# WU-CVGL/CasualHDRSplat

Measured on AMD Instinct MI355X. Metric: train-step images/sec (fwd+bwd raster) @ 1M Gaussians 1080p, higher is better.
Workload: dtype f32; 1 GPU; c3: 1000000 Gaussians, 1920x1080, SH degree 3, HDR radiance + CRF tone-map, 1 pose(s)/view, 1 view(s)/step (one per GPU); num_rendered_R=6777809, R_prime=3025699, pixel_pair_evals_E=559372855, seed=0, binning=sync-free fixed capacity 1.25*R, launch=eager (one enqueue per kernel)

## Files before the change

### casualhdrsplat_amd/csrc/api.hip

```cpp
#include <stdarg.h>
#include <stdio.h>
#include <stdlib.h>
#include <string.h>
#include <time.h>
#include <unistd.h>
#include <atomic>

#include "hs_cloud.h"

namespace hs {

static thread_local char g_err[512] = "";

#ifdef HS_TESTING
int fault_injection() {
    static const int mode = [] {
        const char* e = getenv("HS_FAULT_INJECT");
        return (e && !strcmp(e, "sort_ticket")) ? 1 : (e && !strcmp(e, "stalled_chain")) ? 2 : (e && !strcmp(e, "late_block")) ? 3 : 0;
    }();
    return mode;
}
#endif

static std::atomic<int> g_sort_tickets{0};
// ... 51 lines not shown

void set_error(const char* fmt, ...) {
    va_list ap;
    va_start(ap, fmt);
    vsnprintf(g_err, sizeof g_err, fmt, ap);
    va_end(ap);
}

int64_t crf_partial_floats(int K, int64_t HW, int n_poses);
int64_t pose_partial_floats(int P, int N);

static int plan(const hs_dims& d, hs_sizes* sz, hs_layout* L) {
    if (d.P < 0 || d.W <= 0 || d.H <= 0 || d.n_poses < 1 || d.capacity < 0 || d.M < 0 || d.crf_K < 0 || d.crf_K > 4096 ||
        d.crf_K == 1 || d.n_poses > kMaxPoses) {
        set_error("hs_plan: bad dims P=%d W=%d H=%d N=%d capacity=%lld", d.P, d.W, d.H, d.n_poses, (long long)d.capacity);
        return HS_EINVAL;
    }
    if (d.n_frames < 0 || d.n_frames > d.n_poses || (d.n_frames > 1 && d.n_poses % d.n_frames != 0)) {
        set_error("hs_plan: n_frames=%d must lie in [0, n_poses=%d] and divide n_poses", d.n_frames, d.n_poses);
        return HS_EINVAL;
    }
    const int F = frames_of(d), npf = d.n_poses / F;
    const int64_t I = (int64_t)d.P * d.n_poses;
    const int64_t gx = (d.W + kTile - 1) / kTile, gy = (d.H + kTile - 1) / kTile;
    const int64_t vtiles = gx * gy * d.n_poses;
    if (I >= (1ll << 30) || vtiles >= (1ll << 31) || d.capacity >= (1ll << 30) || gx * gy >= (1ll << 22)) {
        set_error("hs_plan: problem too large (instances and binning capacity must stay below 2^30, tiles per pose below 2^22)");
        return HS_EINVAL;
    }
    const int64_t HW = (int64_t)d.W * d.H;
    hs_layout l;
    int64_t o = 0;
    auto carve = [&o](int64_t bytes) { int64_t at = o; o = align_up(o + bytes, 256); return at; };
    l.counters = carve(sizeof(hs_counters));
    l.rec = carve(I * kRecFloats * 4);
    l.depth = carve(I * 4);
    l.radii = carve(I * 4);
    l.tiles_touched = carve(I * 4);
    l.offsets = carve(I * 4);
    l.cov3D = carve((int64_t)d.P * 6 * 4);
    l.clamped = carve(I);
    l.scan_spine = carve(((I + 255) / 256 + 1) * 4);
    l.binfo = carve(I * 8);
    sz->geom_bytes = o;
    o = 0;
    l.keys_sorted = carve(2 * align_up(d.capacity * 4, 256));
    l.point_list = l.keys_sorted + align_up(d.capacity * 4, 256);
    l.pairs_tmp = carve(d.capacity * 8);
    l.ranges = carve(vtiles * 8);
    l.sort_tmp = carve(sort_tmp_bytes(I));
    l.depth_ws = carve(depth_ws_words(I) * 4);
    l.depth_pairs = carve(2 * I * 8);
    l.inst_sorted = carve(I * 4);
    l.offs_sorted = carve(I * 4);
    l.pair_sort_tmp = carve(emit_scan_words(I) * 4 + sort_tmp_bytes(d.capacity));
    l.pair_flags = carve(d.capacity);
    l.pair_act = carve(d.capacity);
    l.tile_matrix = carve(count_matrix_words(I, vtiles, d.capacity) * 4);
    l.hier_ws = carve(hier_ws_words(I, gx, gy, d.n_poses, d.capacity) * 4);
    sz->binning_bytes = o;
    o = 0;
    l.final_T = carve(HW * d.n_poses * 4);
    l.n_contrib = carve(HW * d.n_poses * 4);
    l.pose_hdr = carve(HW * 3 * 4 * (d.n_poses + (npf > 1 ? F : 0)));
    l.tile_work = carve(vtiles * 4);
    l.tile_order = carve(vtiles * 4);
    sz->image_bytes = o;
    o = 0;
    l.pair_grads = carve(d.capacity * kPairFloats * 4);
    l.crf_partials = carve(crf_partial_floats(d.crf_K, HW, d.n_poses) * 4);
    l.inst_grads = carve(I * kInstFloats * 4);
    l.pose_partials = carve(pose_partial_floats(d.P, d.n_poses) * 4);
    sz->bwd_bytes = o;
    if (L) *L = l;
    return HS_OK;
}

static int debug_sync(int flags, hipStream_t s, const char* stage) {
    if (!(flags & HS_FLAG_DEBUG)) return HS_OK;
    const hipError_t e = hipStreamSynchronize(s);
    if (e != hipSuccess) {
        set_error("debug: stage `%s` failed: %s", stage, hipGetErrorString(e));
        return HS_EHIP;
    }
    return HS_OK;
}

static int check_common(const hs_dims& d, const float* means3D, const float* shs, const float* colors,
                        const float* scales, const float* rots, const float* cov, const float* view,
                        const float* proj, const float* campos, const float* bg, const char* who) {
    if (!means3D || !view || !proj || !campos || !bg) { set_error("%s: null required pointer", who); return HS_EINVAL; }
    if ((shs == nullptr) == (colors == nullptr)) { set_error("%s: provide exactly one of shs / colors_precomp", who); return HS_EINVAL; }
    const bool sr = scales && rots;
    if (sr == (cov != nullptr) || ((scales == nullptr) != (rots == nullptr))) {
        set_error("%s: provide exactly one of (scales, rotations) / cov3D_precomp", who);
        return HS_EINVAL;
    }
    if (shs) {
        if (d.M > 32) {
            set_error("%s: M=%d SH coefficients per channel; at most 32 are supported", who, d.M);
            return HS_EINVAL;
        }
        if (d.sh_degree < 0 || d.sh_degree > 3 || (d.sh_degree + 1) * (d.sh_degree + 1) > d.M) {
            set_error("%s: sh_degree %d needs %d coefficients, M=%d", who, d.sh_degree, (d.sh_degree + 1) * (d.sh_degree + 1), d.M);
            return HS_EINVAL;
        }
    }
// ... 354 lines not shown
```

### casualhdrsplat_amd/csrc/binning.hip

```cpp
#include "hs_common.h"

#ifndef HS_EMIT_NT_MASK
#define HS_EMIT_NT_MASK 6
#endif

namespace hs {

namespace {

constexpr int kScanItems = 4;
constexpr int kScanTile = 256 * kScanItems;

__device__ __forceinline__ uint32_t wave_incl_scan(uint32_t v, int lane) {
#pragma unroll
    for (int d = 1; d < 64; d <<= 1) {
        uint32_t t = __shfl_up(v, d);
        if (lane >= d) v += t;
    }
    return v;
}

template <int NW = 4>
__device__ __forceinline__ uint32_t block_incl_scan(uint32_t v, uint32_t* s_wave , uint32_t* total) {
    const int lane = threadIdx.x & 63, wave = threadIdx.x >> 6;
// ... 1072 lines not shown
                        const int l = (int)__builtin_ctzll(missing);
                        missing &= missing - 1ull;
                        const int q = base - l;
                        uint32_t tot = 0;
                        for (int r = 0; r < 4; ++r) {
                            const int64_t ii = (int64_t)q * 256 + r * 64 + lane;
                            if (ii < I && counters->overflow < 2u) {
                                const uint2 rq = binfo[inst_sorted[ii]];
                                tot += (rq.y & 0xFFFFu) * (rq.y >> 16);
                            }
                        }
#pragma unroll
                        for (int d = 32; d >= 1; d >>= 1) tot += (uint32_t)__shfl_xor((int)tot, d);
                        if (lane == 0) {
                            atomicCAS(reinterpret_cast<unsigned long long*>(scan_status + q), 0ull, (unsigned long long)(kScAgg | (uint64_t)tot));
                            atomicAdd(&counters->reserved[4], 1u);
                        }
                    }
                }
                __builtin_amdgcn_s_sleep(1);
                if ((x & kScFlag) == 0ull) x = sc_read(scan_status + idx);
            }
            const uint64_t flag = x & kScFlag;
            poison = poison || __ballot(flag == 0ull || flag == kScPoison) != 0ull;
            const uint64_t incl_mask = __ballot(flag == kScIncl || flag == kScPoison || flag == 0ull);
            const int first = incl_mask ? (int)__builtin_ctzll(incl_mask) : 64;
            uint64_t v = lane <= first ? (x & ~kScFlag) : 0ull;
#pragma unroll
            for (int d = 32; d >= 1; d >>= 1) v += (uint64_t)__shfl_xor((long long)v, d);
            excl += v;
            if (incl_mask) break;
        }
        if (lane == 0) {
            if (blk != 0) sc_publish(scan_status + blk, (poison ? kScPoison : kScIncl) | ((excl + block_total) & ~kScFlag));
            s_excl = poison ? kScPoison : excl;
        }
    }
    __syncthreads();
    const bool poison = (s_excl & kScFlag) != 0ull;
    const uint64_t bexcl = s_excl & ~kScFlag;
    const uint64_t bend = bexcl + block_total;
    if (blk == (int)gridDim.x - 1 && threadIdx.x == 0) {
        const bool over = bend > capacity;
        counters->num_rendered = bend > 0xFFFFFFFFull ? 0xFFFFFFFFu : (uint32_t)bend;
        if (poison) counters->overflow = 2u;
        else if (over && counters->overflow < 2u) counters->overflow = 1u;
        counters->reserved[0] = (poison || over || counters->overflow != 0u) ? 0u : (uint32_t)bend;
        counters->reserved[5] = COUNT ? (uint32_t)kTileSortCount : (uint32_t)kTileSortRadix;
    }
    uint32_t beg = 0, end = 0;
    end = (uint32_t)bexcl + incl;
    beg = end - cnt;
    if (i < I) offs_sorted[i] = end;
    if (poison || bend > capacity) return;
    if (i < I && end > beg) {
        float* slot_start = &reinterpret_cast<float*>(rec + kRecF4 * (int64_t)inst + 2)[3];
        if constexpr (BIG && (HS_EMIT_NT_MASK & 2)) __builtin_nontemporal_store(__uint_as_float(beg), slot_start);
        else *slot_start = __uint_as_float(beg);
    }
    const uint32_t last_end = __shfl(end, 63 - __builtin_clzll(__ballot(i < I) | 1ull));
    if (i >= I) beg = end = last_end;
    {
        const uint32_t w = rc.y & 0xFFFFu;
        const uint32_t pose = I > (int64_t)P ? inst / (uint32_t)P : 0u;
        const uint32_t key0 = pose * (uint32_t)(gx * gy) + (rc.x >> 16) * (uint32_t)gx + (rc.x & 0xFFFFu);
        s_beg[wave][lane] = beg;
        s_own[wave][lane] = make_uint4(key0, w, __float_as_uint(1.0f / (float)w), inst);
    }
    int sh[4] = {0, 0, 0, 0}, wd[4] = {0, 0, 0, 0};
    {
        int shift = 0;
#pragma unroll
        for (int pass = 0; pass < 4; ++pass) {
            if (pass < passes) {
                const int w = (nbits - shift + (passes - pass) - 1) / (passes - pass);
                sh[pass] = shift; wd[pass] = w;
                shift += w;
            }
        }
    }
    const uint32_t first = __shfl(beg, 0);
    const uint32_t total = last_end - first;
    for (uint32_t p = lane; p < total; p += 64) {
        const uint32_t pos = first + p;
        uint32_t k = 0;
#pragma unroll
        for (uint32_t step = 32; step >= 1; step >>= 1)
            k |= (uint32_t)((int32_t)(s_beg[wave][k + step] - pos - 1u) >> 31) & step;
        const uint4 o = s_own[wave][k];
        const uint32_t t = pos - s_beg[wave][k];
        const uint32_t ty = (uint32_t)(((float)t + 0.5f) * __uint_as_float(o.z));
        const uint32_t tx = t - ty * o.y;
        const uint32_t key = o.x + ty * (uint32_t)gx + tx;
        if constexpr (BIG && (HS_EMIT_NT_MASK & 4)) { __builtin_nontemporal_store(key, &pairs[pos].x); __builtin_nontemporal_store(o.w, &pairs[pos].y); }
        else pairs[pos] = make_uint2(key, o.w);
        pair_flags[pos] = 0;
        if constexpr (COUNT) {
            atomicAdd(&s_hist[key], 1u << (8 * wave));
            continue;
        }
        const uint64_t act = __ballot(true);
#pragma unroll
        for (int pass = 0; pass < 4; ++pass) {
            if (pass < passes) {
                const uint32_t dgt = (key >> sh[pass]) & ((1u << wd[pass]) - 1u);
                const uint32_t d0 = __builtin_amdgcn_readfirstlane(dgt);
// ... 247 lines not shown
    for (int t = threadIdx.x; t < passes * 256; t += 256) s_dig[t] = 0;
    if (blockIdx.x == 0 && threadIdx.x < 2 * kDepthBitsCopies) depth_bits[threadIdx.x] = 0ull;
    const int wave = threadIdx.x >> 6, lane = threadIdx.x & 63;
    const int blk = blockIdx.x;
    const int64_t i = (int64_t)blk * 256 + threadIdx.x;
    uint32_t inst = 0;
    uint2 rc = make_uint2(0u, 0u);
    if (i < I && counters->overflow < 2u) { inst = inst_sorted[i]; rc = srect[i]; }
    const uint32_t cnt = (rc.y & 0xFFFFu) * (rc.y >> 16);
    uint32_t sx0, sy0, sw, sh;
    hier_coarse_rect(rc, sx0, sy0, sw, sh);
    const uint32_t ccnt = sw * sh;
    uint32_t block_total, block_ctotal;
    const uint32_t incl = block_incl_scan(cnt, s_wsum, &block_total);
    const uint32_t cincl = block_incl_scan(ccnt, s_wsum, &block_ctotal);
    if (excl_ready) {
        if (threadIdx.x == 0) { s_excl = block_excl[blk]; s_cexcl = block_cexcl[blk]; }
    } else {
        unsigned long long part = 0, cpart = 0;
        if (super_sums) {
            const int nsup = (HS_ABL & 8) ? 0 : blk / 4;
            for (int j = threadIdx.x; j < nsup; j += 256) { part += super_sums[j]; cpart += super_csums[j]; }
            if ((int)threadIdx.x < blk - 4 * (blk / 4)) { part += block_excl[4 * (blk / 4) + threadIdx.x]; cpart += block_cexcl[4 * (blk / 4) + threadIdx.x]; }
        } else {
            for (int j = threadIdx.x; j < ((HS_ABL & 8) ? 0 : blk); j += 256) { part += block_excl[j]; cpart += block_cexcl[j]; }
        }
#pragma unroll
        for (int d = 32; d >= 1; d >>= 1) {
            part += (unsigned long long)__shfl_xor((long long)part, d);
            cpart += (unsigned long long)__shfl_xor((long long)cpart, d);
        }
        if (lane == 0) { s_wsum64[wave] = part; s_beg[0][wave] = (uint32_t)cpart; }
        __syncthreads();
        if (threadIdx.x == 0) {
            s_excl = (s_wsum64[0] + s_wsum64[1]) + (s_wsum64[2] + s_wsum64[3]);
            s_cexcl = (s_beg[0][0] + s_beg[0][1]) + (s_beg[0][2] + s_beg[0][3]);
        }
    }
    __syncthreads();
    const uint64_t bexcl = s_excl;
    const uint64_t bend = bexcl + block_total;
    const uint32_t cbexcl = s_cexcl;
    if (blk == (int)gridDim.x - 1 && threadIdx.x == 0) {
        const bool over = bend > capacity;
        counters->num_rendered = bend > 0xFFFFFFFFull ? 0xFFFFFFFFu : (uint32_t)bend;
        if (over && counters->overflow < 2u) counters->overflow = 1u;
        const bool empty = over || counters->overflow != 0u;
        counters->reserved[0] = empty ? 0u : (uint32_t)bend;
        counters->reserved[5] = (uint32_t)kTileSortHier;
        hier[0] = empty ? 0u : cbexcl + block_ctotal;
    }
    const uint32_t end = (uint32_t)bexcl + incl, beg = end - cnt;
    if (i < I) offs_sorted[i] = end;
    if (bend > capacity) return;
    if (!(HS_ABL & 1) && i < I && end > beg) {
        float* slot_start = &reinterpret_cast<float*>(rec + kRecF4 * (int64_t)inst + 2)[3];
        if constexpr (BIG && (HS_HIER_NT_MASK & 2)) __builtin_nontemporal_store(__uint_as_float(beg), slot_start);
        else *slot_start = __uint_as_float(beg);
    }
    if (!(HS_ABL & 2)) {
        const uint64_t a0 = min(bend, (bexcl + 15ull) & ~15ull), a1 = max(a0, bend & ~15ull);
        for (uint64_t q = bexcl + threadIdx.x; q < a0; q += 256) pair_flags[q] = 0;
        for (uint64_t q = a0 + 16ull * threadIdx.x; q < a1; q += 16ull * 256) *reinterpret_cast<uint4*>(pair_flags + q) = make_uint4(0u, 0u, 0u, 0u);
        for (uint64_t q = a1 + threadIdx.x; q < bend; q += 256) pair_flags[q] = 0;
    }
    uint32_t cend = cbexcl + cincl, cbeg = cend - ccnt;
    const uint32_t last_end = __shfl(cend, 63 - __builtin_clzll(__ballot(i < I) | 1ull));
    if (i >= I) cbeg = cend = last_end;
    {
        const int sgx = (gx + kSuper - 1) / kSuper, sgy = (gy + kSuper - 1) / kSuper;
        const uint32_t pose = I > (int64_t)P ? inst / (uint32_t)P : 0u;
        const uint32_t key0 = pose * (uint32_t)(sgx * sgy) + sy0 * (uint32_t)sgx + sx0;
        s_beg[wave][lane] = cbeg;
        s_own[wave][lane] = make_uint4(key0 | (sw << 12), rc.x, rc.y, inst);
    }
    const int sgx = (gx + kSuper - 1) / kSuper;
    const uint32_t first = __shfl(cbeg, 0);
    const uint32_t total = last_end - first;
    for (uint32_t p = lane; p < ((HS_ABL & 4) ? 0u : total); p += 64) {
        const uint32_t pos = first + p;
        uint32_t k = 0;
#pragma unroll
        for (uint32_t step = 32; step >= 1; step >>= 1)
            k |= (uint32_t)((int32_t)(s_beg[wave][k + step] - pos - 1u) >> 31) & step;
        const uint4 o = s_own[wave][k];
        const uint32_t t = pos - s_beg[wave][k];
        const uint32_t csw = o.x >> 12;
        const uint32_t cy = (uint32_t)(((float)t + 0.5f) * (1.0f / (float)csw));
        const uint32_t cx = t - cy * csw;
        const uint32_t key = (o.x & 0xFFFu) + cy * (uint32_t)sgx + cx;
        const uint32_t x0 = o.y & 0xFFFFu, y0 = o.y >> 16, x1 = x0 + (o.z & 0xFFFFu), y1 = y0 + (o.z >> 16);
        const uint32_t ox = (x0 / kSuper + cx) * kSuper, oy = (y0 / kSuper + cy) * kSuper;
        const uint32_t lx0 = max(x0, ox) - ox, lx1 = min(x1, ox + kSuper) - ox;
        const uint32_t ly0 = max(y0, oy) - oy, ly1 = min(y1, oy + kSuper) - oy;
        const uint32_t word = key | ((lx0 | (ly0 << 3) | ((lx1 - lx0 - 1u) << 6) | ((ly1 - ly0 - 1u) << 9)) << kb);
        if constexpr (BIG && (HS_HIER_NT_MASK & 4)) { __builtin_nontemporal_store(word, &elems[pos].x); __builtin_nontemporal_store(o.w, &elems[pos].y); }
        else elems[pos] = make_uint2(word, o.w);
        atomicAdd(&s_hist[key], 1u);
    }
    __syncthreads();
    uint32_t* mine = st_count + (int64_t)(blockIdx.x % kHierCopies) * nst_pad;
    for (int t = threadIdx.x; t < nst; t += 256) {
        const uint32_t c = s_hist[t];
        if (c) {
            atomicAdd(&mine[t], c);
            int shift = 0;
// ... 555 lines not shown
```

### casualhdrsplat_amd/csrc/hs_common.h

```cpp
#pragma once
#include <hip/hip_runtime.h>
#include <stdint.h>

#include "../../include/hdrsplat.h"

#if defined(__HIP_DEVICE_COMPILE__) && !defined(__gfx950__)
#error "libhdrsplat is written for gfx950 (MI355X) only: build with --offload-arch=gfx950"
#endif

namespace hs {

void set_error(const char* fmt, ...);

#define HS_HIP_CHECK(expr)                                                                         \
    do {                                                                                           \
        hipError_t e_ = (expr);                                                                    \
        if (e_ != hipSuccess) {                                                                    \
            ::hs::set_error("%s failed: %s (%s:%d)", #expr, hipGetErrorString(e_), __FILE__, __LINE__); \
            return HS_EHIP;                                                                        \
        }                                                                                          \
    } while (0)
#define HS_LAUNCH_CHECK() HS_HIP_CHECK(hipGetLastError())

#ifndef HS_TUNE_CRF_IN_RENDER_TAIL
#define HS_TUNE_CRF_IN_RENDER_TAIL 1
#endif

#ifndef HS_TUNE_COUNT_SORT
#define HS_TUNE_COUNT_SORT 1
#endif

constexpr int kTile = HS_TILE;
constexpr int kRecF4 = 4;
constexpr int kPairF4 = 4;
constexpr int kInstF4 = 4;
constexpr int kRecFloats = 4 * kRecF4;
constexpr int kPairFloats = 4 * kPairF4;
constexpr int kInstFloats = 4 * kInstF4;
constexpr int kSortBlock = 256;
constexpr int kDepthBins = 512, kDepthDigitBits = 9;
#ifndef HS_TUNE_DEPTH_ITEMS
#define HS_TUNE_DEPTH_ITEMS 8
#endif
constexpr int kDepthSortItems = HS_TUNE_DEPTH_ITEMS, kDepthSortLook = 8;
constexpr int kPairSortItems = 16, kPairSortLook = 8;
constexpr int kU64SortItems = 16;
constexpr int kDepthTile = kDepthSortItems * kDepthBins, kPairTile = kPairSortItems * kSortBlock, kU64Tile = kU64SortItems * kSortBlock;
static_assert(kPairTile == kU64Tile && kDepthTile >= kPairTile, "the scratch of every sort is sized for the smallest tile");
constexpr int kSortTileMin = kPairTile;

static inline int64_t align_up(int64_t v, int64_t a) { return (v + a - 1) / a * a; }
static inline int ceil_div(int64_t a, int64_t b) { return (int)((a + b - 1) / b); }
constexpr int kMaxPoses = 21845;
static inline int frames_of(const hs_dims& d) { return d.n_frames > 1 ? d.n_frames : 1; }

static inline int tile_bits(uint32_t n) {
    int b = 0;
    while (n) { ++b; n >>= 1; }
    return b;
}

int launch_preprocess_fwd(const hs_fwd_args& a, const hs_layout& L, hipStream_t s, uint32_t frame_tag);
int launch_scan(const hs_fwd_args& a, const hs_layout& L, hipStream_t s);
int launch_cov3d(const hs_fwd_args& a, const hs_layout& L, hipStream_t s);
struct SortChoice;
int launch_binning(const hs_fwd_args& a, const hs_layout& L, const SortChoice& sort, hipStream_t s, uint32_t frame_tag);
int launch_empty_frame(hs_counters* clear, uint2* ranges, int64_t ntiles, uint32_t* counters_host, const hs_counters* counters,
                       hipStream_t s);
int launch_render_fwd(const hs_fwd_args& a, const hs_layout& L, hipStream_t s, unsigned long long* stats = nullptr);
int launch_render_bwd(const hs_bwd_args& a, const hs_layout& L, hipStream_t s, unsigned long long* stats = nullptr,
                      unsigned long long* timeline = nullptr, bool crf_in_tail = false);
int render_stats_count();
struct CrfReduce;
int launch_crf_bwd(const hs_bwd_args& a, const hs_layout& L, hipStream_t s, CrfReduce* defer, bool in_render_tail = false);
int launch_preprocess_bwd(const hs_bwd_args& a, const hs_layout& L, hipStream_t s, bool segsum, bool project,
                          const CrfReduce* crf_reduce);
int launch_mark_visible(int P, const float* means3D, const float* view, uint8_t* vis, hipStream_t s);
int launch_spline_poses(int J, int T, int kind, const float* delta, const float* base, const float* times, float* w2c,
                        float* jac, int* seg, hipStream_t s);
int launch_sh_backward_views(int P, int M, int deg, int V, const float* means3D, const float* camposes,
                             const float* view_colors, float* d_shs, hipStream_t s);
int64_t loss_pair_count(int planes, int H, int W);
int launch_loss_fwd(const hs_loss_args& a, hipStream_t s);
int launch_loss_bwd(const hs_loss_args& a, hipStream_t s);
int launch_activate_fwd(const hs_activate_args& a, hipStream_t s);
int launch_activate_bwd(const hs_activate_args& a, hipStream_t s);

constexpr int kGhistCopies = 16;
constexpr int kGhistWords = kGhistCopies * 8 * 256;
constexpr int kTicketWords = 128, kDepthBitsAt = 32, kDepthBitsCopies = 16, kDepthBitsWords = 4 * kDepthBitsCopies;
static_assert(kDepthBitsAt >= 8 && kDepthBitsAt % 2 == 0 && kDepthBitsAt + kDepthBitsWords <= kTicketWords, "depth bits live in the ticket row");
__host__ __device__ inline int64_t sweep_pass_words(int64_t nblk, int bins = 256) { return nblk * bins; }
static inline int64_t sort_scratch_words(int64_t n, int passes, int tile, int bins = 256) {
    return n > 0 ? kGhistWords + kTicketWords + (int64_t)passes * sweep_pass_words((n + tile - 1) / tile, bins) : 0;
}
static inline int64_t depth_scratch_words(int64_t I) { return sort_scratch_words(I, 4, kDepthTile, kDepthBins); }
int64_t sort_tmp_bytes(int64_t n);
constexpr int kMsdBits = 12, kMsdBuckets = 1 << kMsdBits;
#ifndef HS_TUNE_MSD_RANGE
#define HS_TUNE_MSD_RANGE 2048
#endif
constexpr int kMsdRange = HS_TUNE_MSD_RANGE, kMsdCap = 4096;
#ifndef HS_TUNE_MSD_SMALL_RANGE
#define HS_TUNE_MSD_SMALL_RANGE 512
#endif
// ... 145 lines not shown
}
__device__ __forceinline__ void depth_bits_accumulate(uint32_t key, bool visible, unsigned long long* bits, uint32_t tag,
                                                      uint32_t* s_two ) {
    depth_bits_accumulate2(visible ? key : 0u, visible ? ~key : 0u, bits, tag, s_two);
}
__device__ __forceinline__ float radiance_dact(int act, float col, bool was_clamped) {
    if (act == 1) return col;
    if (act == 2) return -expm1f(-col);
    return was_clamped ? 0.f : 1.f;
}

struct SegsumArgs {
    int64_t I;
    const uint32_t* inst_sorted; const uint32_t* offs_sorted;
    const float4* pair_grads; const uint8_t* pair_flags; float4* inst_grads; const hs_counters* counters;
    const int* radii_inst; const uint8_t* clamped; float* view_colors; const float4* rec; int act;
};
__device__ __forceinline__ void pair_segsum_body(const SegsumArgs& a, int64_t t) {
    const int64_t i = t >> 2;
    const int q = (int)(t & 3);
    const bool valid = i < a.I && !a.counters->overflow;
    const uint32_t beg = valid ? (i == 0 ? 0u : a.offs_sorted[i - 1]) : 0u;
    const uint32_t end = valid ? a.offs_sorted[i] : 0u;
    float r[10] = {0.f, 0.f, 0.f, 0.f, 0.f, 0.f, 0.f, 0.f, 0.f, 0.f};
    for (uint32_t s = beg + q; s < end; s += 8) {
        const bool two = s + 4 < end;
        const bool f0 = a.pair_flags[s] != 0;
        const bool f1 = two && a.pair_flags[s + 4] != 0;
        float4 a0 = make_float4(0.f, 0.f, 0.f, 0.f), a1 = a0, b0 = a0, b1 = a0;
        float2 a2 = make_float2(0.f, 0.f), b2 = a2;
        if (f0) {
            a0 = a.pair_grads[kPairF4 * (int64_t)s + 0];
            a1 = a.pair_grads[kPairF4 * (int64_t)s + 1];
            a2 = reinterpret_cast<const float2*>(a.pair_grads + kPairF4 * (int64_t)s + 2)[0];
        }
        if (f1) {
            b0 = a.pair_grads[kPairF4 * (int64_t)(s + 4) + 0];
            b1 = a.pair_grads[kPairF4 * (int64_t)(s + 4) + 1];
            b2 = reinterpret_cast<const float2*>(a.pair_grads + kPairF4 * (int64_t)(s + 4) + 2)[0];
        }
        r[0] += a0.x; r[1] += a0.y; r[2] += a0.z; r[3] += a0.w;
        r[4] += a1.x; r[5] += a1.y; r[6] += a1.z; r[7] += a1.w;
        r[8] += a2.x; r[9] += a2.y;
        r[0] += b0.x; r[1] += b0.y; r[2] += b0.z; r[3] += b0.w;
        r[4] += b1.x; r[5] += b1.y; r[6] += b1.z; r[7] += b1.w;
        r[8] += b2.x; r[9] += b2.y;
    }
#pragma unroll
    for (int k = 0; k < 10; ++k) {
        r[k] += __shfl_xor(r[k], 1);
        r[k] += __shfl_xor(r[k], 2);
    }
    if (i < a.I && q == 0) {
        const int64_t inst = a.counters->overflow >= 2u ? i : (int64_t)a.inst_sorted[i];
        float4* o = a.inst_grads + kInstF4 * inst;
        o[0] = make_float4(r[0], r[1], r[2], r[3]);
        o[1] = make_float4(r[4], r[5], r[6], r[7]);
        o[2] = make_float4(r[8], r[9], 0.f, 0.f);
        if constexpr (kInstF4 == 4) o[3] = make_float4(0.f, 0.f, 0.f, 0.f);
        if (a.view_colors) {
            const uint8_t cl = a.clamped[inst];
            const bool on = a.radii_inst[inst] > 0;
            float col[3] = {0.f, 0.f, 0.f};
            if (a.act != 0 && on) {
                const float4 rb = a.rec[kRecF4 * inst + 1];
                col[0] = rb.z; col[1] = rb.w; col[2] = reinterpret_cast<const float*>(a.rec + kRecF4 * inst + 2)[0];
            }
            a.view_colors[3 * inst + 0] = on ? radiance_dact(a.act, col[0], cl & 1) * r[6] : 0.f;
            a.view_colors[3 * inst + 1] = on ? radiance_dact(a.act, col[1], cl & 2) * r[7] : 0.f;
            a.view_colors[3 * inst + 2] = on ? radiance_dact(a.act, col[2], cl & 4) * r[8] : 0.f;
        }
    }
}

__device__ __forceinline__ float xform_row(const float* m, int i, float x, float y, float z) {
    return ((m[i] * x + m[4 + i] * y) + m[8 + i] * z) + m[12 + i];
}

}
```

### casualhdrsplat_amd/csrc/preprocess.hip

```cpp
#include "hs_common.h"


namespace hs {

namespace {

__device__ constexpr float SH_C0 = 0.28209479177387814f;
__device__ constexpr float SH_C1 = 0.4886025119029199f;
__device__ constexpr float SH_C2[5] = {1.0925484305920792f, -1.0925484305920792f, 0.31539156525252005f,
                                       -1.0925484305920792f, 0.5462742152960396f};
__device__ constexpr float SH_C3[7] = {-0.5900435899266435f, 2.890611442640554f, -0.4570457994644658f,
                                       0.3731763325901154f,  -0.4570457994644658f, 1.445305721320277f,
                                       -0.5900435899266435f};

struct Ewa {
    float tx, ty, tz;
    bool clamp_x, clamp_y;
    float a0[3], a1[3];
    float fx, fy;
};

__device__ __forceinline__ void quat_to_R(const float* q, float* R) {
    float r = q[0], x = q[1], y = q[2], z = q[3];
    R[0] = 1.f - 2.f * (y * y + z * z); R[1] = 2.f * (x * y - r * z);       R[2] = 2.f * (x * z + r * y);
// ... 321 lines not shown
        depth_bits_accumulate(depth_key, depth_key != 0xFFFFFFFFu,
                              reinterpret_cast<unsigned long long*>(p.sort_zero + p.bits_at), p.frame_tag, s_two);
        for (int64_t t = lin; t < p.n_vtiles; t += (int64_t)gridDim.x * 256) p.ranges[t] = make_uint2(0u, 0u);
        for (int64_t t = lin; t < p.n_sort_zero; t += (int64_t)gridDim.x * 256)
            if (t < p.bits_at || t >= p.bits_at + kDepthBitsWords) p.sort_zero[t] = 0u;
        for (int64_t t = lin; t < p.n_pair_zero; t += (int64_t)gridDim.x * 256) p.pair_zero[t] = 0u;
        if (lin == 0) {
            p.counters->overflow = 0u;
            p.counters->reserved[1] = (uint32_t)((int64_t)p.P * p.N);
            p.counters->reserved[2] = 0u; p.counters->reserved[3] = 0u;
            p.counters->reserved[4] = 0u;
        }
    }
}

__global__ void __launch_bounds__(256) cov3d_kernel(int P, float mod, const float* scales, const float* rots, const float* cov_pre,
                                                    float* cov3D) {
    const int g = blockIdx.x * 256 + threadIdx.x;
    if (g >= P) return;
    float s6[6];
    if (cov_pre) {
#pragma unroll
        for (int k = 0; k < 6; ++k) s6[k] = cov_pre[6 * (int64_t)g + k];
    } else {
        float sc[3] = {scales[3 * g], scales[3 * g + 1], scales[3 * g + 2]};
        const float4 q4 = reinterpret_cast<const float4*>(rots)[g];
        float q[4] = {q4.x, q4.y, q4.z, q4.w};
        cov3d_from_scale_rot(sc, mod, q, s6);
    }
#pragma unroll
    for (int k = 0; k < 6; ++k) cov3D[6 * (int64_t)g + k] = s6[k];
}

__global__ void mark_visible_kernel(int P, const float* means, const float* V, uint8_t* vis) {
    int i = blockIdx.x * 256 + threadIdx.x;
    if (i >= P) return;
    vis[i] = xform_row(V, 2, means[3 * i], means[3 * i + 1], means[3 * i + 2]) > 0.2f;
}

__global__ void __launch_bounds__(256) pair_segsum_kernel(SegsumArgs sg, CrfReduce crf_reduce) {
    for (int b = blockIdx.x; b < crf_reduce.nblocks; b += gridDim.x) crf_reduce_block(crf_reduce, b);
    pair_segsum_body(sg, (int64_t)blockIdx.x * 256 + threadIdx.x);
}

struct PreBwd {
    int P, M, W, H, N;
    float tanfovx, tanfovy, mod;
    const float* view; const float* proj; const float* campos;
    const float* means; const float* shs; const float* scales; const float* rots; const float* opac;
    bool has_colors_precomp, has_cov_pre, antialias;
    int act;
    const float4* rec; const int* radii_inst; const uint32_t* tiles; const uint32_t* offsets; const float* cov_pre;
    const uint8_t* clamped;
    const float4* inst_grads;
    float* d_means3D; float* d_means2D; float* d_opac; float* d_shs; float* d_colors; float* d_scales;
    float* d_rots; float* d_cov;
    float* dens_grad; float* dens_denom; int* dens_radii;
    int NF;
    float* pose_partials;
    int blk0;
};

constexpr int kPoseVals = 28;

constexpr int kPreBwdBlock = 128;

__device__ __forceinline__ void stage_rows_in(float* s_rows, const float* src, int rows, int M3, int ld) {
    if ((M3 & 3) == 0 && (reinterpret_cast<uintptr_t>(src) & 15) == 0) {
        const int q = M3 >> 2;
        const float4* src4 = reinterpret_cast<const float4*>(src);
        for (int i = threadIdx.x; i < rows * q; i += kPreBwdBlock) {
            const float4 v = src4[i];
            const int r = i / q;
            float* d = s_rows + r * ld + ((i - r * q) << 2);
            d[0] = v.x; d[1] = v.y; d[2] = v.z; d[3] = v.w;
        }
    } else {
        for (int i = threadIdx.x; i < rows * M3; i += kPreBwdBlock) s_rows[(i / M3) * ld + (i % M3)] = src[i];
    }
}
#ifndef HS_TUNE_PB_UNROLL
#define HS_TUNE_PB_UNROLL 1
#endif
template <int Q>
__device__ __forceinline__ void stage_rows_issue(float4 (&v)[Q > 0 ? Q : 1], const float* src) {
    const float4* src4 = reinterpret_cast<const float4*>(src);
#pragma unroll
    for (int j = 0; j < Q; ++j) v[j] = src4[j * kPreBwdBlock + threadIdx.x];
}
template <int Q>
__device__ __forceinline__ void stage_rows_commit(float* s_rows, const float4 (&v)[Q > 0 ? Q : 1], int ld) {
#pragma unroll
    for (int j = 0; j < Q; ++j) {
        const int i = j * kPreBwdBlock + threadIdx.x;
        const int r = i / Q;
        float* d = s_rows + r * ld + ((i - r * Q) << 2);
        d[0] = v[j].x; d[1] = v[j].y; d[2] = v[j].z; d[3] = v[j].w;
    }
}
__device__ __forceinline__ void stage_rows_out(float* dst, const float* s_rows, int rows, int M3, int ld) {
    if ((M3 & 3) == 0 && (reinterpret_cast<uintptr_t>(dst) & 15) == 0) {
        const int q = M3 >> 2;
        float4* dst4 = reinterpret_cast<float4*>(dst);
        for (int i = threadIdx.x; i < rows * q; i += kPreBwdBlock) {
            const int r = i / q;
            const float* sr = s_rows + r * ld + ((i - r * q) << 2);
            typedef float v4f __attribute__((ext_vector_type(4)));
            __builtin_nontemporal_store(v4f{sr[0], sr[1], sr[2], sr[3]}, reinterpret_cast<v4f*>(dst4) + i);
        }
    } else {
        for (int i = threadIdx.x; i < rows * M3; i += kPreBwdBlock) dst[i] = s_rows[(i / M3) * ld + (i % M3)];
    }
}

#ifndef HS_TUNE_PB_WAVES
#define HS_TUNE_PB_WAVES 0
#endif
#if HS_TUNE_PB_WAVES > 0
#define HS_PB_OCC __attribute__((amdgpu_waves_per_eu(HS_TUNE_PB_WAVES, HS_TUNE_PB_WAVES)))
#else
#define HS_PB_OCC
#endif
template <int DEG, bool POSE, bool SHG>
__global__ void __launch_bounds__(kPreBwdBlock) HS_PB_OCC preprocess_bwd_kernel(PreBwd p) {
    extern __shared__ float s_sh[];
    __shared__ float s_pose[kPreBwdBlock / 64][kPoseVals];
    constexpr int NC = (DEG + 1) * (DEG + 1);
    const int blk = (int)blockIdx.x + p.blk0;
    const int g0 = blk * kPreBwdBlock;
    const int g = g0 + threadIdx.x;
    const int M3 = p.M * 3, ld = M3 + 1;
    const int rows = min(kPreBwdBlock, p.P - g0);
    const bool stage_in = !p.has_colors_precomp && DEG >= 1;
    constexpr int Q = (3 * NC) % 4 == 0 && HS_TUNE_PB_UNROLL ? 3 * NC / 4 : 0;
    float4 staged[Q > 0 ? Q : 1];
    bool fast_stage = false;
    if constexpr (Q > 0) {
        const float* src = p.shs + (int64_t)g0 * M3;
        fast_stage = stage_in && M3 == 3 * NC && rows == kPreBwdBlock && (reinterpret_cast<uintptr_t>(src) & 15) == 0;
        if (fast_stage) stage_rows_issue<Q>(staged, src);
    }
    const bool valid = g < p.P;
    const float x = valid ? p.means[3 * g] : 0.f, y = valid ? p.means[3 * g + 1] : 0.f, z = valid ? p.means[3 * g + 2] : 0.f;
    float s6[6] = {0.f, 0.f, 0.f, 0.f, 0.f, 0.f};
    float4 rot4 = make_float4(0.f, 0.f, 0.f, 0.f);
    float scl[3] = {0.f, 0.f, 0.f};
    if (valid) {
        if (p.cov_pre) {
#pragma unroll
            for (int k = 0; k < 6; ++k) s6[k] = p.cov_pre[6 * (int64_t)g + k];
        } else {
            scl[0] = p.scales[3 * g]; scl[1] = p.scales[3 * g + 1]; scl[2] = p.scales[3 * g + 2];
            rot4 = reinterpret_cast<const float4*>(p.rots)[g];
        }
    }
    const int rad0 = valid ? p.radii_inst[g] : 0;
    float4 pre_q0 = make_float4(0.f, 0.f, 0.f, 0.f), pre_q1 = pre_q0;
    float2 pre_q2 = make_float2(0.f, 0.f);
    uint8_t pre_cl = 0;
    if (rad0 > 0) {
        pre_q0 = p.inst_grads[kInstF4 * (int64_t)g + 0]; pre_q1 = p.inst_grads[kInstF4 * (int64_t)g + 1];
        pre_q2 = reinterpret_cast<const float2*>(p.inst_grads + kInstF4 * (int64_t)g + 2)[0];
        if (!p.has_colors_precomp) pre_cl = p.clamped[g];
    }
    if (stage_in) {
        if (fast_stage) { if constexpr (Q > 0) stage_rows_commit<Q>(s_sh, staged, ld); }
        else stage_rows_in(s_sh, p.shs + (int64_t)g0 * M3, rows, M3, ld);
    }
    if (stage_in) __syncthreads();
    float gm[3] = {0.f, 0.f, 0.f};
    float gcov[6] = {0.f, 0.f, 0.f, 0.f, 0.f, 0.f};
    float gm2d[2] = {0.f, 0.f};
    float gop = 0.f;
    float gcol_pre[3] = {0.f, 0.f, 0.f};

    if (valid && !p.cov_pre) {
        const float q[4] = {rot4.x, rot4.y, rot4.z, rot4.w};
        cov3d_from_scale_rot(scl, p.mod, q, s6);
    }

    int max_radius = 0;
    const bool dens_frames = p.dens_grad != nullptr && p.NF < p.N;
    float fm2d[2] = {0.f, 0.f};
    bool frame_on = false;
    int frame_last = p.NF - 1;
    for (int pose = 0; pose < p.N; ++pose) {
        const int64_t idx = (int64_t)pose * p.P + g;
        const int rad = pose == 0 ? rad0 : (valid ? p.radii_inst[idx] : 0);
        const bool on = rad > 0;
        if (on) max_radius = max(max_radius, rad);
        float pg[POSE ? kPoseVals : 1];
        if constexpr (POSE) {
#pragma unroll
            for (int k = 0; k < kPoseVals; ++k) pg[k] = 0.f;
        }
        if (on) {
        float r[9];
        float r9;
        {
            float4 q0 = pre_q0, q1 = pre_q1;
            float2 q2 = pre_q2;
            if (pose != 0) {
                q0 = p.inst_grads[kInstF4 * idx + 0]; q1 = p.inst_grads[kInstF4 * idx + 1];
                q2 = reinterpret_cast<const float2*>(p.inst_grads + kInstF4 * idx + 2)[0];
            }
            r[0] = q0.x; r[1] = q0.y; r[2] = q0.z; r[3] = q0.w; r[4] = q1.x; r[5] = q1.y; r[6] = q1.z; r[7] = q1.w;
            r[8] = q2.x;
            r9 = q2.y;
        }
        gm2d[0] += r[0]; gm2d[1] += r[1];
        if (dens_frames) { fm2d[0] += r[0]; fm2d[1] += r[1]; frame_on = true; }
        if (!p.antialias) gop += r[5];

        const float* V = p.view + 16 * pose;
        const float* PM = p.proj + 16 * pose;
        const float pvx = xform_row(V, 0, x, y, z), pvy = xform_row(V, 1, x, y, z), pvz = xform_row(V, 2, x, y, z);
        Ewa e;
        ewa_setup(V, p.W, p.H, p.tanfovx, p.tanfovy, pvx, pvy, pvz, e);
        float u0[3], u1[3];
        sym_mul(s6, e.a0, u0);
        sym_mul(s6, e.a1, u1);
        const float a = dot3(e.a0, u0) + 0.3f, b = dot3(e.a1, u0), cc = dot3(e.a1, u1) + 0.3f;
        const float denom = a * cc - b * b;
        const float denom2inv = 1.0f / ((denom * denom) + 0.0000001f);
        const float gA = r[2], gB = r[3], gC = r[4];
        float aa_da = 0.f, aa_db = 0.f, aa_dc = 0.f;
        if (p.antialias) {
            const float det0 = (a - 0.3f) * (cc - 0.3f) - b * b;
            const float q = det0 / denom;
            const float sfac = sqrtf(fmaxf(0.000025f, q));
            gop += r[5] * sfac;
            if (q > 0.000025f) {
                const float k = r[5] * p.opac[g] * 0.5f / sfac / (denom * denom);
                aa_da = k * ((cc - 0.3f) * denom - det0 * cc);
                aa_dc = k * ((a - 0.3f) * denom - det0 * a);
                aa_db = k * (2.f * b * (det0 - denom));
            }
        }
        if (denom2inv != 0.f) {
            const float dLda = denom2inv * (-cc * cc * gA + b * cc * gB + (denom - a * cc) * gC) + aa_da;
            const float dLdc = denom2inv * (-a * a * gC + a * b * gB + (denom - a * cc) * gA) + aa_dc;
            const float dLdb = denom2inv * (2.f * b * cc * gA - (denom + 2.f * b * b) * gB + 2.f * a * b * gC) + aa_db;
            const float* pp = e.a0; const float* qq = e.a1;
            gcov[0] += pp[0] * pp[0] * dLda + pp[0] * qq[0] * dLdb + qq[0] * qq[0] * dLdc;
            gcov[3] += pp[1] * pp[1] * dLda + pp[1] * qq[1] * dLdb + qq[1] * qq[1] * dLdc;
            gcov[5] += pp[2] * pp[2] * dLda + pp[2] * qq[2] * dLdb + qq[2] * qq[2] * dLdc;
            gcov[1] += 2.f * pp[0] * pp[1] * dLda + (pp[0] * qq[1] + pp[1] * qq[0]) * dLdb + 2.f * qq[0] * qq[1] * dLdc;
            gcov[2] += 2.f * pp[0] * pp[2] * dLda + (pp[0] * qq[2] + pp[2] * qq[0]) * dLdb + 2.f * qq[0] * qq[2] * dLdc;
            gcov[4] += 2.f * pp[1] * pp[2] * dLda + (pp[1] * qq[2] + pp[2] * qq[1]) * dLdb + 2.f * qq[1] * qq[2] * dLdc;
            float dJ00 = 0.f, dJ02 = 0.f, dJ11 = 0.f, dJ12 = 0.f;
            float ga0v[3], ga1v[3];
#pragma unroll
            for (int j = 0; j < 3; ++j) {
                const float ga0 = 2.f * dLda * u0[j] + dLdb * u1[j];
                const float ga1 = 2.f * dLdc * u1[j] + dLdb * u0[j];
                ga0v[j] = ga0; ga1v[j] = ga1;
                dJ00 += ga0 * V[4 * j + 0]; dJ02 += ga0 * V[4 * j + 2];
// ... 123 lines not shown
            for (int j = 0; j < 3; ++j) Mx[3 * k + j] = s[k] * R[3 * j + k];
        }
        const float G[9] = {gcov[0], 0.5f * gcov[1], 0.5f * gcov[2], 0.5f * gcov[1], gcov[3],
                            0.5f * gcov[4], 0.5f * gcov[2], 0.5f * gcov[4], gcov[5]};
        float dR[9], dsc[3];
#pragma unroll
        for (int k = 0; k < 3; ++k) {
            float ds = 0.f;
#pragma unroll
            for (int j = 0; j < 3; ++j) {
                const float dM = 2.f * ((Mx[3 * k + 0] * G[0 + j] + Mx[3 * k + 1] * G[3 + j]) + Mx[3 * k + 2] * G[6 + j]);
                ds += dM * R[3 * j + k];
                dR[3 * j + k] = s[k] * dM;
            }
            dsc[k] = p.mod * ds;
        }
        const float r = q[0], qx = q[1], qy = q[2], qz = q[3];
        if (p.d_scales) { p.d_scales[3 * g] = dsc[0]; p.d_scales[3 * g + 1] = dsc[1]; p.d_scales[3 * g + 2] = dsc[2]; }
        if (p.d_rots) {
            float4 o;
            o.x = 2.f * (-qz * dR[1] + qy * dR[2] + qz * dR[3] - qx * dR[5] - qy * dR[6] + qx * dR[7]);
            o.y = 2.f * (qy * dR[1] + qz * dR[2] + qy * dR[3] - 2.f * qx * dR[4] - r * dR[5] + qz * dR[6] + r * dR[7] - 2.f * qx * dR[8]);
            o.z = 2.f * (-2.f * qy * dR[0] + qx * dR[1] + r * dR[2] + qx * dR[3] + qz * dR[5] - r * dR[6] + qz * dR[7] - 2.f * qy * dR[8]);
            o.w = 2.f * (-2.f * qz * dR[0] - r * dR[1] + qx * dR[2] + r * dR[3] - 2.f * qz * dR[4] + qy * dR[5] + qx * dR[6] + qy * dR[7]);
            reinterpret_cast<float4*>(p.d_rots)[g] = o;
        }
    } else if (valid && p.d_cov) {
#pragma unroll
        for (int k = 0; k < 6; ++k) p.d_cov[6 * (int64_t)g + k] = gcov[k];
    }
    if (valid && p.dens_grad && max_radius > 0) {
        if (!dens_frames) {
            p.dens_grad[g] += sqrtf(gm2d[0] * gm2d[0] + gm2d[1] * gm2d[1]);
            p.dens_denom[g] += 1.f;
        }
        p.dens_radii[g] = max(p.dens_radii[g], max_radius);
    }
    if (valid) {
        if (p.d_means3D) { p.d_means3D[3 * g] = gm[0]; p.d_means3D[3 * g + 1] = gm[1]; p.d_means3D[3 * g + 2] = gm[2]; }
        if (p.d_means2D) { p.d_means2D[3 * g] = gm2d[0]; p.d_means2D[3 * g + 1] = gm2d[1]; p.d_means2D[3 * g + 2] = 0.f; }
        if (p.d_opac) p.d_opac[g] = gop;
        if (p.has_colors_precomp && p.d_colors) {
            p.d_colors[3 * g] = gcol_pre[0]; p.d_colors[3 * g + 1] = gcol_pre[1]; p.d_colors[3 * g + 2] = gcol_pre[2];
        }
    }
    if constexpr (SHG) {
        if (!p.has_colors_precomp && p.d_shs) {
            float* row = s_sh + threadIdx.x * ld;
            for (int k = 0; k < M3; ++k) row[k] = 0.f;
            if (valid) {
                for (int pose = 0; pose < p.N; ++pose) {
                    const int64_t idx = (int64_t)pose * p.P + g;
                    if ((pose == 0 ? rad0 : p.radii_inst[idx]) <= 0) continue;
                    const float4 q1 = pose == 0 ? pre_q1 : p.inst_grads[kInstF4 * idx + 1];
                    const float q2 = pose == 0 ? pre_q2.x : reinterpret_cast<const float*>(p.inst_grads + kInstF4 * idx + 2)[0];
                    const uint8_t cl = pose == 0 ? pre_cl : p.clamped[idx];
                    float col[3] = {0.f, 0.f, 0.f};
                    if (p.act != 0) {
                        const float4 rb = p.rec[kRecF4 * idx + 1];
                        col[0] = rb.z; col[1] = rb.w; col[2] = reinterpret_cast<const float*>(p.rec + kRecF4 * idx + 2)[0];
                    }
                    const float gc[3] = {radiance_dact(p.act, col[0], cl & 1) * q1.z, radiance_dact(p.act, col[1], cl & 2) * q1.w,
                                         radiance_dact(p.act, col[2], cl & 4) * q2};
                    const float* cp = p.campos + 3 * pose;
                    const float dx = x - cp[0], dy = y - cp[1], dz = z - cp[2];
                    const float len = sqrtf((dx * dx + dy * dy) + dz * dz);
                    float bs[NC];
                    sh_basis<DEG>(dx / len, dy / len, dz / len, bs);
#pragma unroll
                    for (int k = 0; k < NC; ++k) {
                        row[3 * k + 0] += bs[k] * gc[0];
                        row[3 * k + 1] += bs[k] * gc[1];
                        row[3 * k + 2] += bs[k] * gc[2];
                    }
                }
            }
            __syncthreads();
            float* dst = p.d_shs + (int64_t)g0 * M3;
            stage_rows_out(dst, s_sh, rows, M3, ld);
        }
    }
}

template <int DEG>
__global__ void __launch_bounds__(kPreBwdBlock) sh_views_kernel(int P, int M, int V, const float* means, const float* campos,
                                                                const float* view_colors, float* d_shs) {
    extern __shared__ float s_sh[];
    constexpr int NC = (DEG + 1) * (DEG + 1);
    const int g0 = blockIdx.x * kPreBwdBlock;
    const int g = g0 + threadIdx.x;
    const int M3 = M * 3, ld = M3 + 1;
    const int rows = min(kPreBwdBlock, P - g0);
    float gsh[NC * 3];
#pragma unroll
    for (int k = 0; k < NC * 3; ++k) gsh[k] = 0.f;
    if (g < P) {
        const float x = means[3 * g], y = means[3 * g + 1], z = means[3 * g + 2];
        for (int v = 0; v < V; ++v) {
            const float* gcp = view_colors + 3 * ((int64_t)v * P + g);
            const float gc[3] = {gcp[0], gcp[1], gcp[2]};
            const float* cp = campos + 3 * v;
            const float dx = x - cp[0], dy = y - cp[1], dz = z - cp[2];
            const float len = sqrtf((dx * dx + dy * dy) + dz * dz);
            const float ux = dx / len, uy = dy / len, uz = dz / len;
            float bs[NC];
            sh_basis<DEG>(ux, uy, uz, bs);
#pragma unroll
            for (int k = 0; k < NC; ++k) {
// ... 68 lines not shown
    p.means = a.means3D; p.opac = a.opacities; p.shs = a.shs; p.colors = a.colors_precomp; p.scales = a.scales;
    p.rots = a.rotations; p.cov_pre = a.cov3D_precomp;
    p.rec = (float4*)(geom + L.rec); p.depth = (float*)(geom + L.depth); p.radii_inst = (int*)(geom + L.radii);
    p.tiles = (uint32_t*)(geom + L.tiles_touched); p.cov3D = (float*)(geom + L.cov3D);
    p.clamped = (uint8_t*)(geom + L.clamped); p.radii_out = a.radii;
    p.binfo = (uint2*)(geom + L.binfo);
    p.antialias = (a.flags & HS_FLAG_ANTIALIAS) != 0;
    p.act = (a.flags & HS_FLAG_RADIANCE_EXP) ? 1 : (a.flags & HS_FLAG_RADIANCE_SOFTPLUS) ? 2 : 0;
    p.depth_pairs = nullptr; p.counters = nullptr; p.ranges = nullptr; p.n_vtiles = 0;
    p.sort_zero = nullptr; p.n_sort_zero = 0; p.bits_at = 0; p.frame_tag = 0u;
    p.pair_zero = nullptr; p.n_pair_zero = 0;
    if ((a.stages & HS_STAGE_BIN) && a.binning) {
        char* bin = (char*)a.binning;
        p.depth_pairs = (uint2*)(bin + L.depth_pairs);
        p.counters = (hs_counters*)(geom + L.counters); p.ranges = (uint2*)(bin + L.ranges);
        p.n_vtiles = (int64_t)((d.W + kTile - 1) / kTile) * ((d.H + kTile - 1) / kTile) * d.n_poses;
        p.sort_zero = (uint32_t*)(bin + L.sort_tmp);
        p.n_sort_zero = depth_scratch_words((int64_t)d.P * d.n_poses);
        p.bits_at = kGhistWords + kDepthBitsAt;
        p.frame_tag = frame_tag;
        p.pair_zero = (uint32_t*)(bin + L.pair_sort_tmp);
        p.n_pair_zero = pair_scratch_words((int64_t)d.P * d.n_poses, d.capacity,
                                           sort_passes(tile_bits((uint32_t)p.n_vtiles)));
    }
    if (d.n_poses > 1 && d.P > 0) fill_i32_kernel<<<ceil_div((int64_t)d.P, 1024), 256, 0, s>>>(a.radii, (int64_t)d.P, 0);
    const int grid = (int)(ceil_div(ceil_div((int64_t)d.P, 256), 8) * 8 * d.n_poses);
    const int deg = a.colors_precomp ? 0 : d.sh_degree;
    switch (deg) {
        case 0: preprocess_fwd_kernel<0><<<grid, 256, 0, s>>>(p); break;
        case 1: preprocess_fwd_kernel<1><<<grid, 256, 0, s>>>(p); break;
        case 2: preprocess_fwd_kernel<2><<<grid, 256, 0, s>>>(p); break;
        default: preprocess_fwd_kernel<3><<<grid, 256, 0, s>>>(p); break;
    }
    HS_LAUNCH_CHECK();
    return HS_OK;
}

int launch_preprocess_bwd(const hs_bwd_args& a, const hs_layout& L, hipStream_t s, bool segsum, bool project,
                          const CrfReduce* crf_reduce) {
    const hs_dims& d = a.dims;
    const char* geom = (const char*)a.geom;
    PreBwd p;
    p.P = d.P; p.M = d.M; p.W = d.W; p.H = d.H; p.N = d.n_poses;
    p.tanfovx = a.tanfovx; p.tanfovy = a.tanfovy; p.mod = a.scale_modifier;
    p.view = a.viewmatrices; p.proj = a.projmatrices; p.campos = a.camposes;
    p.means = a.means3D; p.shs = a.shs; p.scales = a.scales; p.rots = a.rotations; p.opac = a.opacities;
    p.antialias = (a.flags & HS_FLAG_ANTIALIAS) != 0;
    p.act = (a.flags & HS_FLAG_RADIANCE_EXP) ? 1 : (a.flags & HS_FLAG_RADIANCE_SOFTPLUS) ? 2 : 0;
    p.has_colors_precomp = a.colors_precomp != nullptr; p.has_cov_pre = a.cov3D_precomp != nullptr;
    p.rec = (const float4*)(geom + L.rec); p.radii_inst = (const int*)(geom + L.radii);
    p.tiles = (const uint32_t*)(geom + L.tiles_touched); p.offsets = (const uint32_t*)(geom + L.offsets);
    p.cov_pre = a.cov3D_precomp; p.clamped = (const uint8_t*)(geom + L.clamped);
    p.inst_grads = (const float4*)((const char*)a.bwd + L.inst_grads);
    const CrfReduce no_reduce{nullptr, 0, 0, 0, nullptr, nullptr, 0};
    if (segsum) {
        const int64_t I = (int64_t)d.P * d.n_poses;
        const char* bin = (const char*)a.binning;
        SegsumArgs sg;
        sg.I = I; sg.inst_sorted = (const uint32_t*)(bin + L.inst_sorted); sg.offs_sorted = (const uint32_t*)(bin + L.offs_sorted);
        sg.pair_grads = (const float4*)((const char*)a.bwd + L.pair_grads); sg.pair_flags = (const uint8_t*)bin + L.pair_flags;
        sg.inst_grads = (float4*)((char*)a.bwd + L.inst_grads); sg.counters = (const hs_counters*)(geom + L.counters);
        sg.radii_inst = p.radii_inst; sg.clamped = p.clamped;
        sg.view_colors = a.colors_precomp ? nullptr : a.dL_dview_colors; sg.rec = p.rec; sg.act = p.act;
        pair_segsum_kernel<<<ceil_div(4 * I, 256), 256, 0, s>>>(sg, crf_reduce ? *crf_reduce : no_reduce);
        HS_LAUNCH_CHECK();
    }
    if (!project) return HS_OK;
    p.d_means3D = a.dL_dmeans3D; p.d_means2D = a.dL_dmeans2D; p.d_opac = a.dL_dopacities; p.d_shs = a.dL_dshs;
    p.d_colors = a.dL_dcolors_precomp; p.d_scales = a.dL_dscales; p.d_rots = a.dL_drotations;
    p.d_cov = a.dL_dcov3D_precomp;
    p.dens_grad = a.densify_grad_accum; p.dens_denom = a.densify_denom; p.dens_radii = a.densify_max_radii;
    p.NF = d.n_poses / frames_of(d);
    const bool shg = p.d_shs != nullptr;
    const bool ranged = a.g_begin != 0 || a.g_end != 0;
    const int g_lo = ranged ? a.g_begin : 0, g_hi = ranged ? a.g_end : d.P;
    const int nblk_all = ceil_div(d.P, kPreBwdBlock);
    const int grid = ceil_div(g_hi - g_lo, kPreBwdBlock);
    p.blk0 = g_lo / kPreBwdBlock;
    const int deg = a.colors_precomp ? 0 : d.sh_degree;
    const size_t lds = (size_t)kPreBwdBlock * (d.M * 3 + 1) * sizeof(float);
    float* pose_partials = a.dL_dviewmatrices ? (float*)((char*)a.bwd + L.pose_partials) : nullptr;
    p.pose_partials = pose_partials;
#define HS_LAUNCH_PRE_BWD(DEG_)                                                                              \
    if (pose_partials && shg) preprocess_bwd_kernel<DEG_, true, true><<<grid, kPreBwdBlock, lds, s>>>(p);       \
    else if (pose_partials) preprocess_bwd_kernel<DEG_, true, false><<<grid, kPreBwdBlock, lds, s>>>(p);        \
    else if (shg) preprocess_bwd_kernel<DEG_, false, true><<<grid, kPreBwdBlock, lds, s>>>(p);                  \
    else preprocess_bwd_kernel<DEG_, false, false><<<grid, kPreBwdBlock, lds, s>>>(p)
    if (grid > 0) switch (deg) {
        case 0: HS_LAUNCH_PRE_BWD(0); break;
        case 1: HS_LAUNCH_PRE_BWD(1); break;
        case 2: HS_LAUNCH_PRE_BWD(2); break;
        default: HS_LAUNCH_PRE_BWD(3); break;
    }
#undef HS_LAUNCH_PRE_BWD
    HS_LAUNCH_CHECK();
    if (pose_partials && g_hi >= d.P) {
        const int grid = nblk_all;
        const int cols = d.n_poses * kPoseVals;
        float* stage = pose_partials + (int64_t)grid * cols;
        pose_reduce1_kernel<<<dim3(ceil_div(cols, 256), kPoseChunks), 256, 0, s>>>(pose_partials, grid, cols, stage);
        pose_reduce2_kernel<<<ceil_div(d.n_poses * 35, 256), 256, 0, s>>>(stage, d.n_poses, a.dL_dviewmatrices,
                                                                        a.dL_dprojmatrices, a.dL_dcamposes);
        HS_LAUNCH_CHECK();
    }
    return HS_OK;
}
// ... 34 lines not shown
```

Before: 967.9 images/s.

## Store per-instance gradients in sorted order and gather them via an inverse rank map

```diff
diff --git a/casualhdrsplat_amd/csrc/api.hip b/casualhdrsplat_amd/csrc/api.hip
--- a/casualhdrsplat_amd/csrc/api.hip
+++ b/casualhdrsplat_amd/csrc/api.hip
@@ -127,7 +127,7 @@
     l.depth_ws = carve(depth_ws_words(I) * 4);
     l.depth_pairs = carve(2 * I * 8);
     l.inst_sorted = carve(I * 4);
-    l.offs_sorted = carve(I * 4);
+    l.offs_sorted = carve((inst_rank_words_behind_offs(I) + I) * 4);
     l.pair_sort_tmp = carve(emit_scan_words(I) * 4 + sort_tmp_bytes(d.capacity));
     l.pair_flags = carve(d.capacity);
     l.pair_act = carve(d.capacity);
diff --git a/casualhdrsplat_amd/csrc/binning.hip b/casualhdrsplat_amd/csrc/binning.hip
--- a/casualhdrsplat_amd/csrc/binning.hip
+++ b/casualhdrsplat_amd/csrc/binning.hip
@@ -1148,6 +1148,7 @@
     end = (uint32_t)bexcl + incl;
     beg = end - cnt;
     if (i < I) offs_sorted[i] = end;
+    if (i < I && counters->overflow < 2u) (offs_sorted + inst_rank_words_behind_offs(I))[inst] = (uint32_t)i;
     if (poison || bend > capacity) return;
     if (i < I && end > beg) {
         float* slot_start = &reinterpret_cast<float*>(rec + kRecF4 * (int64_t)inst + 2)[3];
@@ -1501,6 +1502,7 @@
     }
     const uint32_t end = (uint32_t)bexcl + incl, beg = end - cnt;
     if (i < I) offs_sorted[i] = end;
+    if (i < I && counters->overflow < 2u) (offs_sorted + inst_rank_words_behind_offs(I))[inst] = (uint32_t)i;
     if (bend > capacity) return;
     if (!(HS_ABL & 1) && i < I && end > beg) {
         float* slot_start = &reinterpret_cast<float*>(rec + kRecF4 * (int64_t)inst + 2)[3];
diff --git a/casualhdrsplat_amd/csrc/hs_common.h b/casualhdrsplat_amd/csrc/hs_common.h
--- a/casualhdrsplat_amd/csrc/hs_common.h
+++ b/casualhdrsplat_amd/csrc/hs_common.h
@@ -51,6 +51,7 @@
 
 static inline int64_t align_up(int64_t v, int64_t a) { return (v + a - 1) / a * a; }
 static inline int ceil_div(int64_t a, int64_t b) { return (int)((a + b - 1) / b); }
+__host__ __device__ static inline int64_t inst_rank_words_behind_offs(int64_t I) { return (I * 4 + 255) / 256 * 64; }
 constexpr int kMaxPoses = 21845;
 static inline int frames_of(const hs_dims& d) { return d.n_frames > 1 ? d.n_frames : 1; }
 
@@ -302,13 +303,13 @@
         r[k] += __shfl_xor(r[k], 2);
     }
     if (i < a.I && q == 0) {
-        const int64_t inst = a.counters->overflow >= 2u ? i : (int64_t)a.inst_sorted[i];
-        float4* o = a.inst_grads + kInstF4 * inst;
+        float4* o = a.inst_grads + kInstF4 * i;
         o[0] = make_float4(r[0], r[1], r[2], r[3]);
         o[1] = make_float4(r[4], r[5], r[6], r[7]);
         o[2] = make_float4(r[8], r[9], 0.f, 0.f);
         if constexpr (kInstF4 == 4) o[3] = make_float4(0.f, 0.f, 0.f, 0.f);
         if (a.view_colors) {
+            const int64_t inst = a.counters->overflow >= 2u ? i : (int64_t)a.inst_sorted[i];
             const uint8_t cl = a.clamped[inst];
             const bool on = a.radii_inst[inst] > 0;
             float col[3] = {0.f, 0.f, 0.f};
diff --git a/casualhdrsplat_amd/csrc/preprocess.hip b/casualhdrsplat_amd/csrc/preprocess.hip
--- a/casualhdrsplat_amd/csrc/preprocess.hip
+++ b/casualhdrsplat_amd/csrc/preprocess.hip
@@ -397,7 +397,7 @@
     int act;
     const float4* rec; const int* radii_inst; const uint32_t* tiles; const uint32_t* offsets; const float* cov_pre;
     const uint8_t* clamped;
-    const float4* inst_grads;
+    const float4* inst_grads; const uint32_t* inst_rank; uint32_t n_inst;
     float* d_means3D; float* d_means2D; float* d_opac; float* d_shs; float* d_colors; float* d_scales;
     float* d_rots; float* d_cov;
     float* dens_grad; float* dens_denom; int* dens_radii;
@@ -500,12 +500,16 @@
         }
     }
     const int rad0 = valid ? p.radii_inst[g] : 0;
+    const uint32_t slot0 = valid ? p.inst_rank[g] : p.n_inst;
     float4 pre_q0 = make_float4(0.f, 0.f, 0.f, 0.f), pre_q1 = pre_q0;
     float2 pre_q2 = make_float2(0.f, 0.f);
     uint8_t pre_cl = 0;
     if (rad0 > 0) {
-        pre_q0 = p.inst_grads[kInstF4 * (int64_t)g + 0]; pre_q1 = p.inst_grads[kInstF4 * (int64_t)g + 1];
-        pre_q2 = reinterpret_cast<const float2*>(p.inst_grads + kInstF4 * (int64_t)g + 2)[0];
+        if (slot0 < p.n_inst) {
+            const float4* row = p.inst_grads + kInstF4 * (int64_t)slot0;
+            pre_q0 = row[0]; pre_q1 = row[1];
+            pre_q2 = reinterpret_cast<const float2*>(row + 2)[0];
+        }
         if (!p.has_colors_precomp) pre_cl = p.clamped[g];
     }
     if (stage_in) {
@@ -532,6 +536,7 @@
     for (int pose = 0; pose < p.N; ++pose) {
         const int64_t idx = (int64_t)pose * p.P + g;
         const int rad = pose == 0 ? rad0 : (valid ? p.radii_inst[idx] : 0);
+        const uint32_t slot = pose == 0 || !valid ? p.n_inst : p.inst_rank[idx];
         const bool on = rad > 0;
         if (on) max_radius = max(max_radius, rad);
         float pg[POSE ? kPoseVals : 1];
@@ -546,8 +551,12 @@
             float4 q0 = pre_q0, q1 = pre_q1;
             float2 q2 = pre_q2;
             if (pose != 0) {
-                q0 = p.inst_grads[kInstF4 * idx + 0]; q1 = p.inst_grads[kInstF4 * idx + 1];
-                q2 = reinterpret_cast<const float2*>(p.inst_grads + kInstF4 * idx + 2)[0];
+                q0 = make_float4(0.f, 0.f, 0.f, 0.f); q1 = q0; q2 = make_float2(0.f, 0.f);
+                if (slot < p.n_inst) {
+                    const float4* row = p.inst_grads + kInstF4 * (int64_t)slot;
+                    q0 = row[0]; q1 = row[1];
+                    q2 = reinterpret_cast<const float2*>(row + 2)[0];
+                }
             }
             r[0] = q0.x; r[1] = q0.y; r[2] = q0.z; r[3] = q0.w; r[4] = q1.x; r[5] = q1.y; r[6] = q1.z; r[7] = q1.w;
             r[8] = q2.x;
@@ -777,8 +786,16 @@
                 for (int pose = 0; pose < p.N; ++pose) {
                     const int64_t idx = (int64_t)pose * p.P + g;
                     if ((pose == 0 ? rad0 : p.radii_inst[idx]) <= 0) continue;
-                    const float4 q1 = pose == 0 ? pre_q1 : p.inst_grads[kInstF4 * idx + 1];
-                    const float q2 = pose == 0 ? pre_q2.x : reinterpret_cast<const float*>(p.inst_grads + kInstF4 * idx + 2)[0];
+                    float4 q1 = pre_q1;
+                    float q2 = pre_q2.x;
+                    if (pose != 0) {
+                        const uint32_t slot = p.inst_rank[idx];
+                        q1 = make_float4(0.f, 0.f, 0.f, 0.f); q2 = 0.f;
+                        if (slot < p.n_inst) {
+                            const float4* row = p.inst_grads + kInstF4 * (int64_t)slot;
+                            q1 = row[1]; q2 = reinterpret_cast<const float*>(row + 2)[0];
+                        }
+                    }
                     const uint8_t cl = pose == 0 ? pre_cl : p.clamped[idx];
                     float col[3] = {0.f, 0.f, 0.f};
                     if (p.act != 0) {
@@ -953,6 +970,8 @@
     p.tiles = (const uint32_t*)(geom + L.tiles_touched); p.offsets = (const uint32_t*)(geom + L.offsets);
     p.cov_pre = a.cov3D_precomp; p.clamped = (const uint8_t*)(geom + L.clamped);
     p.inst_grads = (const float4*)((const char*)a.bwd + L.inst_grads);
+    p.n_inst = (uint32_t)((int64_t)d.P * d.n_poses);
+    p.inst_rank = (const uint32_t*)((const char*)a.binning + L.offs_sorted) + inst_rank_words_behind_offs(p.n_inst);
     const CrfReduce no_reduce{nullptr, 0, 0, 0, nullptr, nullptr, 0};
     if (segsum) {
         const int64_t I = (int64_t)d.P * d.n_poses;
```

Measured after the change: 978.4 images/s (median of 5 runs). 1.01x the previous value.
